# It4innovations/hyperqueue

Measured on AMD Instinct MI355X. Metric: tasks_assigned_per_sec, higher is better.
Workload: dtype u64

## Files before the change

### hyperqueue_amd/csrc/debug_capi.cpp

```cpp
#include "../../include/hqtick_debug.h"

#include <algorithm>
#include <cstring>

#include "clock_core.h"
#include "hb_order.h"
#include "milp.h"
#include "price_emul.h"

static thread_local int g_last_canonical = 0;
static thread_local long g_last_hull[2] = {0, 0};
extern "C" int hqtick_debug_milp_was_canonical(void) { return g_last_canonical; }
extern "C" void hqtick_debug_milp_last_hull(long *solves, long *nonpacking) {
    if (solves) *solves = g_last_hull[0];
    if (nonpacking) *nonpacking = g_last_hull[1];
}

extern "C" int hqtick_debug_milp_solve(int ncols, const double *obj, const uint8_t *col_kind, int nrows, const uint8_t *row_type,
                                       const double *rhs, const int *row_off, const int *row_col, const double *row_coef,
                                       double time_limit_s, int canonical, double *x_out, double *obj_out, int *is_optimal,
                                       long *nodes_out) {
    hqmilp::Model m;
    m.obj.assign(obj, obj + ncols);
    m.kind.assign(col_kind, col_kind + ncols);
// ... 38 lines not shown
    if (min_cols) emu.min_cols = min_cols;
    hqmilp::Result r = hqmilp::solve(m, time_limit_s, true, hqmilp::REFERENCE_MIP_REL_GAP, use_sweeps ? &emu : nullptr);
    g_last_canonical = r.canonical ? 1 : 0;
    g_last_hull[0] = r.hull_solves; g_last_hull[1] = r.hull_solves_nonpacking;
    if (stats_out) { stats_out[0] = r.price_sweeps; stats_out[1] = r.price_rounds; stats_out[2] = r.price_total_us; stats_out[3] = r.canonical ? 1.0 : 0.0; }
    if (!r.feasible) return 0;
    for (int j = 0; j < ncols; j++) x_out[j] = r.x[j];
    *obj_out = r.objective;
    *is_optimal = r.optimal ? 1 : 0;
    return 1;
}

static thread_local hqmilp::Probe g_block_run_probe;
extern "C" void hqtick_debug_set_block_runs(int on) {
    hqmilp::g_probe = on < 0 ? nullptr : &g_block_run_probe; hqmilp::set_block_runs(on);
    if (on >= 0) { g_block_run_probe.model = g_block_run_probe.tables = g_block_run_probe.runs = g_block_run_probe.covered = 0; }
}
extern "C" void hqtick_debug_corrupt_block_runs(int on) { g_block_run_probe.corrupt_runs = on != 0; }
extern "C" void hqtick_debug_last_coupled_digest(uint64_t out[4]) {
    out[0] = g_block_run_probe.model; out[1] = g_block_run_probe.tables; out[2] = g_block_run_probe.runs; out[3] = g_block_run_probe.covered;
}
extern "C" void hqtick_debug_set_early_sweep(int on) { hqprice::set_early_sweep(on); }
extern "C" uint32_t hqtick_debug_early_sweeps(void) { return hqprice::early_sweeps(); }
extern "C" void hqtick_debug_capture_first_cut(int on) { hqprice::capture_first_cut(on != 0); }
extern "C" uint32_t hqtick_debug_first_cut(unsigned char *out, uint32_t cap) {
    const std::vector<unsigned char> &b = hqprice::first_cut_bytes();
    if (out && cap) memcpy(out, b.data(), std::min<size_t>(cap, b.size()));
    return (uint32_t)b.size();
}

extern "C" int hqtick_debug_clock_rows(uint32_t n, const int64_t *deadline_ns, int64_t now_ns, uint32_t nv, const uint64_t *min_time_ns, int sorted_form, int64_t *remaining_out) {
    if ((n && (!deadline_ns || !remaining_out)) || (nv && !min_time_ns)) return HQTICK_E_INVALID;
    if (!sorted_form) {
        for (uint32_t w = 0; w < n; w++) {
            if (deadline_ns[w] == hqclock::NO_LIMIT) { remaining_out[w] = hqclock::NO_LIMIT; continue; }
            const int64_t r = hqclock::sat_sub(deadline_ns[w], now_ns);
            uint64_t best = 0;
            for (uint32_t v0 = 0; r >= 0 && v0 < nv; v0 += hqclock::CHUNK) best = hqclock::fold_thresholds(best, r, min_time_ns + v0, std::min(hqclock::CHUNK, nv - v0));
            remaining_out[w] = r < 0 ? -1 : (int64_t)best;
        }
        return 0;
    }
    std::vector<uint64_t> thr(min_time_ns, min_time_ns + nv);
    std::sort(thr.begin(), thr.end()); thr.erase(std::unique(thr.begin(), thr.end()), thr.end());
    for (uint32_t w = 0; w < n; w++) remaining_out[w] = hqclock::canonical_sorted(deadline_ns[w], now_ns, thr.data(), (uint32_t)thr.size());
    return 0;
// ... 4 lines not shown
```

### hyperqueue_amd/csrc/price.cpp

```cpp
#include "price.h"

#include <algorithm>
#include <chrono>
#include <cmath>
#include <cstdio>
#include <cstdlib>
#include <cstring>
#include <functional>
#include <map>
#include <numeric>

#include "lp_tab.h"
#include "milp.h"

namespace hqprice {
namespace {

using hqmilp::lp::BASIC;
using hqmilp::lp::INF;
using hqmilp::lp::LP_OPT;
using hqmilp::lp::Rows;
using hqmilp::lp::Tab;

constexpr int KMAX_HOST = 128;
constexpr int NMAX_BLOCK = 32, MMAX_BLOCK = 4;
constexpr double FIRST_PROPOSAL_SCALE = 1.0 / 16.0;
constexpr double GRID = 10000.0;
constexpr int MAX_ROUNDS = 6;
constexpr int BP_MAX_NODES = 600;
constexpr double BP_MAX_STEPS = 3.0e6;
constexpr double BP_MAX_WORK = 3.0e9;

double now_us() { return std::chrono::duration<double, std::micro>(std::chrono::steady_clock::now().time_since_epoch()).count(); }
thread_local uint32_t g_early_sweeps = 0;

struct CapRow { int flat; double rhs; std::vector<std::pair<int, double>> g; };

struct Prob {
    HostTables T;
    std::vector<int> flat_of, model_of;
    std::vector<int> gmodel;
    std::vector<double> gcost;
    int K = 0, G = 0;
    std::vector<double> h;
    std::vector<uint8_t> ge;
    std::vector<std::vector<std::pair<int, double>>> g_rows;
    std::vector<int> grp_of;
    int KG = 0;
    std::vector<int> g_off, g_col; std::vector<int32_t> g_coef;
    std::vector<int> gr_off, gr_row;
    size_t row_terms = 0;
    std::vector<CapRow> caps;
    std::vector<int32_t> base_cap;
    std::vector<int> block_of_flat;
    int n_runs = 0, run_blocks = 0;
};

// ... 179 lines not shown
    P.grp_of.assign(P.K, -1);
    std::vector<int> rep;
    for (int k = 0; k < P.K; k++) {
        int g = -1;
        for (size_t i = 0; i < rep.size() && g < 0; i++) if (sig[rep[i]] == sig[k] && wide[rep[i]].cols == wide[k].cols) g = (int)i;
        if (g < 0) { g = (int)rep.size(); rep.push_back(k); }
        P.grp_of[k] = g;
    }
    P.KG = (int)rep.size();
    if (P.KG > KMAX_HOST) return "more than 128 distinct wide left-hand sides";
    std::vector<std::vector<std::pair<int, int32_t>>> lhs((size_t)P.KG);
    for (int g = 0; g < P.KG; g++) lhs[(size_t)g] = std::move(wide[rep[g]].cols);
    finish_groups(P, lhs);
    P.base_cap = T.col_cap;
    return nullptr;
}

struct Cut {
    double cx = 0, bnd = 0; std::vector<long long> act; std::vector<double> pi;
    std::vector<uint16_t> x; bool fetched = false; std::vector<std::pair<uint32_t, int32_t>> lo;
    std::vector<double> pcx; std::vector<long long> pact;
};

struct BPNode { std::vector<int8_t> flag; std::vector<std::pair<uint32_t, int32_t>> lo, hi; double bound = INF; int depth = 0; };

struct Solver {
    const Request &rq; Sweeper &sw; Prob P;
    std::vector<Cut> cuts;
    double relaxed_bound = INF;
    std::vector<double> relaxed_pi;
    double theta_scale = 1.0;
    std::vector<double> pmax;
    bool failed = false;
    size_t cut_lo = 0;
    double work = 0.0;
    double sweep_steps = 0.0; int budget_sweeps = 0;
    int max_sweeps = 256;
    std::vector<std::pair<uint32_t, int32_t>> node_lo, node_caps; double node_cl = 0.0; std::vector<double> node_Al; bool at_root = true;
    bool base_caps = true;
    enum { EARLY_NONE = 0, EARLY_LAUNCHED, EARLY_REFUSED, EARLY_FAILED };
    int early = EARLY_NONE;
    bool early_begun = false;
    bool host_acts = false;
    double tp0 = 0.0;
    Solver(const Request &r, Sweeper &s) : rq(r), sw(s) {}

    void prepare_sweeper() {
        sw.stat_sweeps = 0; sw.stat_sweep_us = 0;
        sw.guard_s = rq.deadline_s - 0.3 * rq.time_limit_s; sw.time_up = false;
        max_sweeps = (int)std::min<size_t>(4096, std::max<size_t>(256, ((size_t)64 << 20) / ((size_t)P.T.n_cols * 2 + 1)));
    }
    void launch_on_blocks() {
        prepare_sweeper();
        const int took = sw.begin_blocks(P.T, (uint32_t)max_sweeps);
        if (took < 0) return;
        if (took == 0) { early = EARLY_REFUSED; return; }
        early_begun = true;
        const double zero = 0.0, t0 = now_us();
        sw.pending_k = 0;
        if (!sw.sweep_launch(&zero)) { early = EARLY_FAILED; return; }
        sw.stat_sweep_us += now_us() - t0;
        early = EARLY_LAUNCHED; host_acts = true; g_early_sweeps++;
        if (rq.trace) fprintf(stderr, "[price] first sweep (prices 0) launched on the block tables at %.3f ms\n", (now_us() - tp0) / 1e3);
    }
    bool activities_from_patterns(uint32_t sweep, SweepTotals &tot) {
        const HostTables &T = P.T;
        const uint16_t *x = sw.patterns(sweep, 1);
// ... 231 lines not shown
                for (size_t k = cut_lo; k < cuts.size(); k++) for (int p = 0; p < NP; p++) {
                    const double l = lam[k * PARTS + p];
                    if (l == 0.0) continue;
                    const long long *pa = &cuts[k].pact[(size_t)p * K];
                    for (int r = 0; r < K; r++) colact[r] += l * (double)pa[r];
                }
                auto keep = std::move(probe); probe = nullptr;
                const bool go = keep(colact, lb_master);
                probe = std::move(keep);
                if (go) return false;
            }
            bool same = !pi_prev_master.empty();
            for (int i = 0; i < KL && same; i++) same = std::fabs(mt.x[i] - pi_prev_master[i]) <= 1e-15 + 1e-12 * std::fabs(mt.x[i]);
            pi_prev_master.assign(mt.x.begin(), mt.x.begin() + KL);
            const double alpha = (it < 3 || same) ? 0.0 : 0.3;
            for (int k = 0; k < K; k++) pi[k] = alpha * pi_best[k];
            for (int i = 0; i < KL; i++) pi[lk[i]] += (1.0 - alpha) * mt.x[i];
            if (it == 0 && cut_lo == 0 && cuts.size() == 1) {
                std::vector<double> pa;
                static const bool agg_on = !(getenv("HQPRICE_AGG_START") && atoi(getenv("HQPRICE_AGG_START")) == 0);
                if (agg_on && aggregate_prices(hB, lk, pa)) { pi = pa; if (rq.trace) fprintf(stderr, "[price]   first proposal: the duals of the model aggregated over chunks of blocks\n"); }
                else for (int k = 0; k < K; k++) pi[k] *= FIRST_PROPOSAL_SCALE;
            }
            const int ci = evaluate(pi);
            if (ci < 0) break;
            if (sw.time_up) { if (rq.trace) fprintf(stderr, "[price] 70 %% of the time limit gone inside the master loop\n"); return false; }
            if (budget_sweeps >= 8) { if (rq.trace) fprintf(stderr, "[price] blocks keep running out of their search budget (%d sweeps): not a model for the sweeps\n", budget_sweeps); return false; }
            const double L = fixed_value(cuts[ci], hB, cB);
            if (L < ub_best) { ub_best = L; pi_best = pi; }
            push_cuts(&mt);
        }
        if (!converged) {
            if (mt.solve(200000) != LP_OPT) return false;
            lb_master = -mt.objective() * theta_scale + cB;
            if (ub_best - lb_master > 1e-3 * std::fabs(ub_best)) { if (rq.trace) fprintf(stderr, "[price] master not converged: %.9f vs %.9f\n", ub_best, lb_master); return false; }
        }
        multipliers(lambda);
        if (rq.trace) fprintf(stderr, "[price]   master: %d priced rows + %d parts, %d cut rows, %ld pivots, %.1f us inside the LP (%d active rows)\n", KL, NP, M.m, mt.iters, lp_us, mt.ma);
        pi_out.assign(K, 0.0);
        for (int i = 0; i < KL; i++) pi_out[lk[i]] = mt.x[i];
        *bound_out = ub_best;
        if (no_sweeps) { settled.valid = true; settled.hB = hB; settled.cB = cB; settled.lambda = lambda; settled.pi = pi_out; settled.bound = ub_best; settled.n_cuts = cuts.size(); settled.cut_lo = cut_lo; }
        return true;
    }

    bool fetch_patterns() {
        size_t first = cuts.size();
        for (size_t k = 0; k < cuts.size(); k++) if (!cuts[k].fetched) { first = k; break; }
        if (first == cuts.size()) return true;
        const uint32_t count = (uint32_t)(cuts.size() - first);
        const uint16_t *pat = sw.patterns((uint32_t)first, count);
        if (!pat) { failed = true; return false; }
        const uint32_t nc = P.T.n_cols;
        for (uint32_t i = 0; i < count; i++) {
            Cut &c = cuts[first + i];
            if (c.fetched) continue;
            c.x.assign(pat + (size_t)i * nc, pat + (size_t)(i + 1) * nc);
            for (auto &l : c.lo) c.x[l.first] = (uint16_t)(c.x[l.first] + l.second);
            c.fetched = true;
        }
        return true;
    }

    std::vector<uint16_t> round_patterns(const std::vector<double> &lambda, const std::vector<double> &pi, const std::vector<double> &hB,
                                         const std::vector<char> *usable = nullptr, const std::vector<int32_t> *lo_of = nullptr, int variant = 0) {
        const int K = P.K; const HostTables &T = P.T;
        const uint32_t S = (uint32_t)cuts.size();
        const double t_r0 = now_us();
        if (!fetch_patterns()) return {};
        auto pat_of = [&](int k) { return cuts[(size_t)k].x.data(); };
        const uint32_t per = (T.n_blocks + PARTS - 1) / PARTS;
        auto lam = [&](int k, uint32_t p) { return lambda[(size_t)k * PARTS + p]; };
        std::vector<int> active;
        for (uint32_t k = 0; k < S; k++) {
            if (usable && !(*usable)[k]) continue;
            bool any = false; for (uint32_t p = 0; p < (uint32_t)PARTS && !any; p++) any = lam((int)k, p) > 1e-9;
            if (any) active.push_back((int)k);
        }
        if (active.empty()) return {};
        const int Q = (int)active.size();
        std::vector<double> lpact(K, 0.0), wgt(K);
        for (int k : active) {
            const Cut &c = cuts[k];
            if (c.pact.empty()) { for (int r = 0; r < K; r++) lpact[r] += lam(k, 0) * (double)c.act[r]; continue; }
            for (uint32_t p = 0; p < (uint32_t)PARTS; p++) { const double l = lam(k, p); if (l > 0.0) for (int r = 0; r < K; r++) lpact[r] += l * (double)c.pact[(size_t)p * P.K + r]; }
        }
        for (int r = 0; r < K; r++) {
            const bool tight = pi[r] > 1e-12 || hB[r] - lpact[r] <= 1e-6 * std::max(1.0, std::fabs(hB[r]));
            wgt[r] = (tight ? 1.0 : 0.02) / std::max(1.0, std::fabs(hB[r]));
        }
        auto block_act = [&](uint32_t b, const uint16_t *x, std::vector<double> &out) {
            double ga[KMAX_HOST];
            for (int g = 0; g < P.KG; g++) ga[g] = 0.0;
            for (uint32_t f = T.blk_off[b]; f < T.blk_off[b + 1]; f++) { const uint16_t xv = x[f]; if (!xv) continue; for (uint32_t e = T.col_woff[f]; e < T.col_woff[f + 1]; e++) ga[T.w_row[e]] += (double)T.w_coef[e] * (double)xv; }
            for (int r = 0; r < K; r++) out[r] = ga[P.grp_of[r]];
        };
        std::vector<uint16_t> x(T.n_cols, 0);
        std::vector<double> cum(K, 0.0);
        std::vector<int> chosen(T.n_blocks, 0);
        {
            const int KG = P.KG;
            std::vector<double> wg(KG, 0.0), cumg(KG, 0.0), tgtg(KG, 0.0), candg((size_t)Q * KG);
            for (int r = 0; r < K; r++) wg[P.grp_of[r]] += wgt[r];
            std::vector<char> on(Q); std::vector<const double *> cgp(Q, nullptr);
            for (uint32_t bi = 0; bi < T.n_blocks; bi++) {
                const uint32_t b = variant == 1 ? T.n_blocks - 1 - bi : bi;
                const uint32_t part = b / per;
                int first = -1; bool all_same = true;
                const size_t blk_bytes = (size_t)(T.blk_off[b + 1] - T.blk_off[b]) * 2;
                for (int q = 0; q < Q; q++) {
                    const double l = lam(active[q], part);
                    on[q] = l > 1e-9;
                    if (!on[q]) continue;
                    const uint16_t *px = pat_of(active[q]);
                    if (first >= 0 && memcmp(px + T.blk_off[b], pat_of(active[first]) + T.blk_off[b], blk_bytes) == 0) cgp[q] = cgp[first];
                    else {
                        if (first < 0) first = q; else all_same = false;
                        double *cg = &candg[(size_t)q * KG];
                        for (int g = 0; g < KG; g++) cg[g] = 0.0;
                        for (uint32_t f = T.blk_off[b]; f < T.blk_off[b + 1]; f++) { const uint16_t xv = px[f]; if (!xv) continue; for (uint32_t e = T.col_woff[f]; e < T.col_woff[f + 1]; e++) cg[T.w_row[e]] += (double)T.w_coef[e] * (double)xv; }
                        cgp[q] = cg;
                    }
                    const double *cg = cgp[q];
                    for (int g = 0; g < KG; g++) tgtg[g] += l * cg[g];
                }
                int bq = -1; double be = INF;
                if (all_same) bq = first;
                else for (int q = 0; q < Q; q++) {
                    if (!on[q]) continue;
                    const double *cg = cgp[q];
                    double e = 0.0;
                    for (int g = 0; g < KG; g++) e += std::fabs(cumg[g] + cg[g] - tgtg[g]) * wg[g];
                    if (e < be - 1e-15) { be = e; bq = q; }
                }
                if (bq < 0) return {};
                const double *cb = cgp[bq];
                for (int g = 0; g < KG; g++) cumg[g] += cb[g];
                chosen[b] = active[bq];
                memcpy(&x[T.blk_off[b]], pat_of(active[bq]) + T.blk_off[b], (size_t)(T.blk_off[b + 1] - T.blk_off[b]) * 2);
            }
            for (int r = 0; r < K; r++) cum[r] = cumg[P.grp_of[r]];
        }
        if (rq.trace) fprintf(stderr, "[price]   rounding: diffusion done at %.3f us, %d active cuts\n", now_us() - t_r0, Q);
        auto ge_short = [&](const std::vector<double> &c) { double s = 0.0; for (int r = 0; r < K; r++) if (P.ge[r] && c[r] > hB[r] + 1e-9) s += c[r] - hB[r]; return s; };
        if (ge_short(cum) > 0.0) {
            std::vector<int> pool = active;
            for (int k = (int)S - 1; k >= 0 && (int)pool.size() < Q + 12; k--) if ((!usable || (*usable)[k]) && std::find(pool.begin(), pool.end(), k) == pool.end()) pool.push_back(k);
            std::vector<double> a0(K), a1(K), c2(K);
            double cmax = 0.0; for (double c : T.col_cost) cmax = std::max(cmax, c);
            struct Cand { double score; uint32_t b; int k; };
            std::vector<Cand> cl; std::vector<double> colshort, coltight;
            auto evaluate_switch = [&](uint32_t b, int k, double v0, double &score) {
                const uint16_t *px = pat_of(k);
                block_act(b, px, a1);
                double gain = 0.0, newviol = 0.0;
                for (int r = 0; r < K; r++) {
                    if (a0[r] == a1[r]) continue;
                    const double c = cum[r] - a0[r] + a1[r];
                    if (P.ge[r]) gain += std::max(0.0, cum[r] - hB[r]) - std::max(0.0, c - hB[r]);
                    else newviol += std::max(0.0, c - hB[r]) - std::max(0.0, cum[r] - hB[r]);
                }
                if (!(gain > 1e-9)) return false;
                double v1 = 0.0; for (uint32_t f = T.blk_off[b]; f < T.blk_off[b + 1]; f++) v1 += T.col_cost[f] * (double)px[f];
                score = gain * 10.0 * cmax - (v0 - v1) - std::max(0.0, newviol) * cmax;
                return true;
            };
            auto value_of = [&](uint32_t b) { double v = 0.0; for (uint32_t f = T.blk_off[b]; f < T.blk_off[b + 1]; f++) v += T.col_cost[f] * (double)x[f]; return v; };
            for (int pass = 0; pass < 64 && ge_short(cum) > 0.0; pass++) {
                const double base = ge_short(cum);
                cl.clear();
                std::vector<int> short_in(P.KG, 0);
                for (int r = 0; r < K; r++) if (P.ge[r] && cum[r] > hB[r] + 1e-9) short_in[P.grp_of[r]]++;
                std::vector<int> tight_in(P.KG, 0);
                double spare = 0.0;
                for (int r = 0; r < K; r++) if (P.ge[r] && cum[r] <= hB[r] + 1e-9 && hB[r] - cum[r] <= 2.0 + 1e-9) { tight_in[P.grp_of[r]]++; spare += std::max(0.0, hB[r] - cum[r]); }
                colshort.assign(T.n_cols, 0.0); coltight.assign(T.n_cols, 0.0);
                for (uint32_t f = 0; f < T.n_cols; f++) for (uint32_t e = T.col_woff[f]; e < T.col_woff[f + 1]; e++) {
                    const int ns = short_in[T.w_row[e]], nt = tight_in[T.w_row[e]];
                    if (ns) colshort[f] += (double)ns * (double)T.w_coef[e];
                    if (nt) coltight[f] += (double)nt * (double)T.w_coef[e];
                }
                for (uint32_t b = 0; b < T.n_blocks; b++) {
                    for (int k : pool) {
                        if (k == chosen[b]) continue;
                        const uint16_t *px = pat_of(k);
                        double gain = 0.0, dv = 0.0, dmg = 0.0; bool differs = false;
                        for (uint32_t f = T.blk_off[b]; f < T.blk_off[b + 1]; f++) {
                            const int d = (int)px[f] - (int)x[f];
                            if (!d) continue;
                            differs = true; dv += T.col_cost[f] * (double)d;
                            gain -= colshort[f] * (double)d;
                            dmg += coltight[f] * (double)d;
                        }
                        if (!differs || !(gain - std::max(0.0, dmg - spare) > 1e-9)) continue;
                        cl.push_back({std::min(gain, base) * 10.0 * cmax + dv, b, k});
                    }
                }
                if (rq.trace) fprintf(stderr, "[price]     pass %d: short by %.1f, %zu candidate switches, at %.3f us\n", pass, base, cl.size(), now_us() - t_r0);
                if (cl.empty()) break;
                const size_t top = std::min<size_t>(cl.size(), 512);
                std::partial_sort(cl.begin(), cl.begin() + (long)top, cl.end(), [](const Cand &p, const Cand &q) { return p.score > q.score || (p.score == q.score && (p.b < q.b || (p.b == q.b && p.k < q.k))); });
                cl.resize(top);
                std::vector<char> moved(T.n_blocks, 0);
                for (const Cand &cd : cl) {
                    if (!(ge_short(cum) > 0.0)) break;
                    if (moved[cd.b]) continue;
                    {
                        const uint16_t *px = pat_of(cd.k); double gain = 0.0;
                        for (uint32_t f = T.blk_off[cd.b]; f < T.blk_off[cd.b + 1]; f++) {
                            const int d = (int)px[f] - (int)x[f];
                            if (d) for (uint32_t e = T.col_woff[f]; e < T.col_woff[f + 1]; e++) { const int g = T.w_row[e]; for (int q = P.gr_off[g]; q < P.gr_off[g + 1]; q++) { const int r = P.gr_row[q]; if (P.ge[r] && cum[r] > hB[r] + 1e-9) gain -= (double)T.w_coef[e] * (double)d; } }
                        }
                        if (!(gain > 1e-9)) continue;
                    }
                    block_act(cd.b, pat_of(chosen[cd.b]), a0);
                    double score;
                    if (!evaluate_switch(cd.b, cd.k, value_of(cd.b), score)) continue;
                    for (int r = 0; r < K; r++) cum[r] += a1[r] - a0[r];
                    chosen[cd.b] = cd.k; moved[cd.b] = 1;
                    memcpy(&x[T.blk_off[cd.b]], pat_of(cd.k) + T.blk_off[cd.b], (size_t)(T.blk_off[cd.b + 1] - T.blk_off[cd.b]) * 2);
                }
                if (ge_short(cum) >= base - 1e-9) break;
            }
            if (ge_short(cum) > 0.0) return {};
        }
        if (rq.trace) fprintf(stderr, "[price]   rounding: >= repair done at %.3f us\n", now_us() - t_r0);
        for (int r = 0; r < K; r++) {
            if (cum[r] <= hB[r] + 1e-9) continue;
            std::vector<int> cols;
            const int gr = P.grp_of[r];
            for (int k = P.g_off[gr]; k < P.g_off[gr + 1]; k++) if (P.g_coef[k] > 0 && x[P.g_col[k]] > 0) cols.push_back(k);
            std::sort(cols.begin(), cols.end(), [&](int a, int b) { const double ca = T.col_cost[P.g_col[a]] / P.g_coef[a], cb = T.col_cost[P.g_col[b]] / P.g_coef[b]; return ca < cb || (ca == cb && a > b); });
            for (int k : cols) {
                const int f = P.g_col[k];
                while (x[f] > (lo_of ? (uint16_t)(*lo_of)[f] : 0) && cum[r] > hB[r] + 1e-9) {
                    bool ok = true;
                    for (uint32_t e = T.col_woff[f]; e < T.col_woff[f + 1] && ok; e++) if (T.w_coef[e] < 0) { const int g = T.w_row[e]; for (int q = P.gr_off[g]; q < P.gr_off[g + 1] && ok; q++) if (cum[P.gr_row[q]] - (double)T.w_coef[e] > hB[P.gr_row[q]] + 1e-9) ok = false; }
                    if (!ok) break;
                    x[f]--;
                    for (uint32_t e = T.col_woff[f]; e < T.col_woff[f + 1]; e++) { const int g = T.w_row[e]; for (int q = P.gr_off[g]; q < P.gr_off[g + 1]; q++) cum[P.gr_row[q]] -= (double)T.w_coef[e]; }
                }
                if (cum[r] <= hB[r] + 1e-9) break;
            }
            if (cum[r] > hB[r] + 1e-9) return {};
        }
        return x;
    }

    struct NodeLP { double bound = INF; bool pruned = false; std::vector<double> lambda, pi, bfrac; };

    bool apply_node(const BPNode &nd, std::vector<int32_t> &lo_arr, std::vector<int32_t> &hi_arr) {
// ... 893 lines not shown
    S.tp0 = tp0;
    if (g_capture_cut) g_first_cut.clear();
    std::vector<double> ub, c; double cmax = 1.0;
    const std::function<void()> hook = [&S]() { S.launch_on_blocks(); };
    if (const char *why = build_from_model(mv, S.P, ub, c, cmax, early_sweep_on() ? &hook : nullptr)) {
        if (S.early_begun) sw.end();
        Answer ans; ans.why = why; return ans;
    }
    if (cost_scale) *cost_scale = cmax;
    Polisher pol(S.P, mv.n);
    rq.polish = [&pol](std::vector<double> &x, double &value) { return pol.run(x, value); };
    return run_solver(S, tp0);
}

void flatten_for_probe(const ModelView &mv, bool trace) {
    Prob P; std::vector<double> ub, c; double cmax = 1.0;
    const char *why = build_from_model(mv, P, ub, c, cmax);
    if (trace) fprintf(stderr, "[price] flattened for the probe alone: %s\n", why ? why : "tables built");
}

void set_check_hints(bool on) { g_check_hints = on; g_hint_mismatches = 0; }
void set_early_sweep(int on) { g_early_sweep = on; g_early_sweeps = 0; }
uint32_t early_sweeps() { return g_early_sweeps; }
void capture_first_cut(bool on) { g_capture_cut = on; g_first_cut.clear(); }
const std::vector<unsigned char> &first_cut_bytes() { return g_first_cut; }
int hint_mismatches() { return g_hint_mismatches; }

Answer solve(const Request &rq, Sweeper &sw) {
    Solver S(rq, sw);
    const double tp0 = now_us();
    if (const char *why = build(rq, S.P)) { Answer ans; ans.why = why; return ans; }
    return run_solver(S, tp0);
}

}
```

### hyperqueue_amd/csrc/price.h

```cpp
#pragma once
#include <cstdint>
#include <functional>
#include <vector>

namespace hqprice {

struct HostTables {
    uint32_t n_blocks = 0, n_cols = 0, K = 0;
    std::vector<uint32_t> blk_off; std::vector<uint8_t> blk_m; std::vector<double> blk_cap;
    std::vector<double> col_cost, col_a; std::vector<int32_t> col_cap; std::vector<uint32_t> col_woff; std::vector<uint16_t> w_row; std::vector<int32_t> w_coef;
};

struct SweepTotals {
    double cx = 0, rc = 0, bnd = 0;
    uint32_t n_budget = 0, max_steps = 0;
    std::vector<long long> act;
    std::vector<double> part_cx;
    std::vector<long long> part_act;
};
constexpr int PARTS = 16;

struct RangeValues { const double *cx = nullptr, *rc = nullptr, *bnd = nullptr; const uint32_t *steps = nullptr; const long long *part_act = nullptr; };

void totals_from_blocks(uint32_t n_blocks, uint32_t K, const double *cx, const double *rc, const double *bnd, const uint32_t *steps, const long long *part_act, SweepTotals &out);

struct Sweeper {
    virtual ~Sweeper() {}
    virtual bool begin(const HostTables &t, uint32_t max_sweeps) = 0;
    virtual int begin_blocks(const HostTables &t, uint32_t max_sweeps) { (void)t; (void)max_sweeps; return -1; }
    virtual bool begin_wide() { return false; }
    virtual bool set_caps(const int32_t *col_cap) = 0;
    virtual bool set_block_caps(const double *blk_cap) = 0;
    virtual bool sweep(const double *pi, SweepTotals &out) = 0;
    virtual bool sweep_launch(const double *pi) { pending_pi.assign(pi, pi + pending_k); return true; }
    virtual bool sweep_finish(SweepTotals &out) { return sweep(pending_pi.data(), out); }
    std::vector<double> pending_pi; uint32_t pending_k = 0;
    virtual const uint16_t *patterns(uint32_t first, uint32_t count) = 0;
    virtual void end() = 0;
    virtual bool sweep_range(const double *pi, uint32_t b0, uint32_t b1, RangeValues &out) { (void)pi; (void)b0; (void)b1; (void)out; return false; }
    double guard_s = 1e300;
    bool time_up = false;
    virtual bool merges_clock() const { return false; }
    uint32_t min_cols = 256;
    uint32_t budget = 4096;
    uint32_t stat_sweeps = 0;
    double stat_sweep_us = 0;
};

struct Request {
    int n = 0, m = 0;
    const int *roff = nullptr, *rcol = nullptr; const double *rcoef = nullptr, *rlo = nullptr, *rhi = nullptr;
    const double *row_scale = nullptr; const uint8_t *row_implied = nullptr;
    const int32_t *col_group = nullptr;
    const double *c = nullptr, *ub = nullptr;
    const double *incumbent = nullptr; double incumbent_value = 0.0;
    double rel_gap = 1e-4;
    double time_limit_s = 5.0;
    double deadline_s = 1e300;
    std::function<bool(std::vector<double> &x, double &value)> polish;
    bool trace = false;
// ... 8 lines not shown
    const char *why = "";
    std::vector<int> block_of; std::vector<double> block_value, rcost;
};

Answer solve(const Request &rq, Sweeper &sw);

struct ModelView {
    int n = 0, m = 0;
    const double *obj = nullptr; const uint8_t *kind = nullptr;
    const uint8_t *rtype = nullptr; const double *rhs = nullptr;
    const int *roff = nullptr, *rcol = nullptr; const double *rcoef = nullptr;
    const int32_t *col_group = nullptr; const uint8_t *row_implied = nullptr;
    const int32_t *row_lhs = nullptr, *row_lhs_len = nullptr;
    const int *list_off = nullptr, *list_col = nullptr; int n_lists = 0;
    const int32_t *row_block = nullptr; const uint32_t *col_ub = nullptr;
    const int32_t *block_runs = nullptr; int n_block_runs = 0;
    uint64_t *run_stats = nullptr;
    uint64_t *tables_digest = nullptr;
};
void set_check_hints(bool on);
int hint_mismatches();
void set_early_sweep(int on);
uint32_t early_sweeps();
void capture_first_cut(bool on);
const std::vector<unsigned char> &first_cut_bytes();
void flatten_for_probe(const ModelView &mv, bool trace);
Answer solve_model(const ModelView &mv, double rel_gap, double time_limit_s, double deadline_s, bool trace, Sweeper &sw, double *cost_scale);

struct Exchange {
    uint32_t rank = 0, world = 1;
    virtual ~Exchange() {}
    virtual bool allgather(const void *send, void *recv, size_t bytes) = 0;
    uint64_t n_calls = 0, n_bytes = 0; double us = 0;
};

struct ShardedSweeper : Sweeper {
    Sweeper &inner; Exchange &ex;
    const HostTables *T = nullptr;
    std::vector<uint32_t> rank_b0, rank_b1, rank_p0, rank_p1;
    uint32_t max_blocks = 0, max_parts = 0, max_cols = 0;
    std::vector<unsigned char> send, recv;
    std::vector<double> cx, rc, bnd; std::vector<uint32_t> steps; std::vector<long long> part_act;
    std::vector<uint16_t> pats;
    uint32_t n_sweeps = 0;
    uint32_t min_blocks = 1025;
    bool pass = false;
// ... 12 lines not shown
```

### hyperqueue_amd/csrc/price_dev.h

```cpp
#pragma once
#include <hip/hip_runtime.h>

#include <cstdlib>

#include "devbuf.h"
#include "price.h"

namespace hqprice {

struct DeviceSweeper : Sweeper {
    hipStream_t stream = nullptr;
    hqbuf::PinBuf h_stage, h_res, h_pats, h_pin, h_prof, h_blkv;
    static constexpr uint32_t PIN_SWEEPS = 64;
    bool sync_clean = false;
    bool in_flight = false; double flight_t0 = 0; uint32_t flight_blocks = 0;
    bool profile = getenv("HQTICK_PRICE_PROFILE") != nullptr; double prof_med[16] = {0}, prof_max[16] = {0}, prof_steps = 0, prof_span = 0, prof_tail = 0; int prof_n = 0;
    hqbuf::DevBuf d_tab, d_pats, d_blk, d_sync, d_prof;
    const HostTables *T = nullptr;
    size_t o_off = 0, o_m = 0, o_cap = 0, o_cost = 0, o_a = 0, o_ccap = 0, o_woff = 0, o_wrow = 0, o_wcoef = 0, tab_bytes = 0;
    bool blocks_only = false;
    uint32_t flight_k = 0;
    size_t wide_room = 0;
    uint32_t n_sweeps = 0, cap_sweeps = 0, seq = 0;
    uint32_t max_block_cols = 0;
    bool force_nmax = getenv("HQTICK_PRICE_NMAX") != nullptr;
    int force_waves = getenv("HQTICK_PRICE_WAVES") ? atoi(getenv("HQTICK_PRICE_WAVES")) : 0;
    uint32_t dbg = getenv("HQTICK_PRICE_DBG") ? (uint32_t)atoi(getenv("HQTICK_PRICE_DBG")) : 0u;
    double last_kernel_us = 0;
    uint64_t total_sweeps = 0, total_block_solves = 0; double total_us = 0;
    explicit DeviceSweeper(hipStream_t s) : stream(s) {}
    ~DeviceSweeper() override;
    bool begin(const HostTables &t, uint32_t max_sweeps) override;
    int begin_blocks(const HostTables &t, uint32_t max_sweeps) override;
    bool begin_wide() override;
    bool size_buffers(const HostTables &t, uint32_t max_sweeps);
    void stage_blocks(const HostTables &t);
    bool set_caps(const int32_t *col_cap) override;
    bool set_block_caps(const double *blk_cap) override;
    bool sweep(const double *pi, SweepTotals &out) override;
    bool sweep_range(const double *pi, uint32_t b0, uint32_t b1, RangeValues &out) override;
    bool launch(const double *pi, uint32_t b0, uint32_t b1, bool local, SweepTotals *out);
    bool launch_only(const double *pi, uint32_t b0, uint32_t b1, bool local);
    bool wait_done(SweepTotals *out);
    bool sweep_launch(const double *pi) override;
    bool sweep_finish(SweepTotals &out) override;
    const uint16_t *patterns(uint32_t first, uint32_t count) override;
    void end() override;
};

}
```

### hyperqueue_amd/csrc/price_emul.h

```cpp
#pragma once
#include <algorithm>
#include <vector>

#include "price.h"

namespace hqprice {

struct EmulatedSweeper : Sweeper {
    const HostTables *T = nullptr;
    std::vector<int32_t> caps;
    std::vector<double> bcaps;
    std::vector<uint16_t> pats;
    std::vector<double> blk_cx, blk_rc, blk_bnd;
    std::vector<uint32_t> blk_steps;
    std::vector<long long> slots;
    uint32_t n_sweeps = 0, cap_sweeps = 0;
    int fail_at = -1;
    bool blocks_only = false, held_there = false;
    std::vector<uint32_t> zero_woff;
    SweepTotals held;
    bool begin(const HostTables &t, uint32_t max_sweeps) override;
    int begin_blocks(const HostTables &t, uint32_t max_sweeps) override;
    bool begin_wide() override;
    bool sweep_launch(const double *pi) override;
    bool sweep_finish(SweepTotals &out) override;
    bool set_caps(const int32_t *col_cap) override;
    bool set_block_caps(const double *blk_cap) override;
    bool sweep(const double *pi, SweepTotals &out) override;
    bool sweep_range(const double *pi, uint32_t b0, uint32_t b1, RangeValues &out) override;
    const uint16_t *patterns(uint32_t first, uint32_t count) override;
    void end() override;
};

}
```

### include/hqtick_debug.h

```cpp
#ifndef HQTICK_DEBUG_H
#define HQTICK_DEBUG_H
#include <stdint.h>
#include "hqtick.h"
#ifdef __cplusplus
extern "C" {
#endif
#if defined(__GNUC__)
#pragma GCC visibility push(default)
#endif

int hqtick_debug_milp_solve(int ncols, const double *obj, const uint8_t *col_kind, int nrows, const uint8_t *row_type,
                            const double *rhs, const int *row_off, const int *row_col, const double *row_coef,
                            double time_limit_s, int canonical, double *x_out, double *obj_out, int *is_optimal,
                            long *nodes_out);

int hqtick_debug_last_order(const hqtick_ctx *ctx, uint32_t *n_runs, uint32_t *n_levels, double *order_us);

int hqtick_debug_last_scan(const hqtick_ctx *ctx, int which, uint32_t *n_levels, uint32_t *n_groups, uint32_t shape[4],
                           uint64_t *levels, uint32_t cap_levels, uint32_t *hist, uint32_t cap_groups);

int hqtick_debug_order_view(hqtick_ctx *ctx, uint32_t n_requests, uint32_t counts[4], uint32_t *perm, uint32_t *inv, uint32_t *lrank, uint64_t cap_slots, uint32_t *run_rq,
                            uint32_t *run_start, uint32_t *run_rank, uint64_t *run_prio, uint32_t cap_runs);
int hqtick_debug_order_select(hqtick_ctx *ctx, const uint32_t *rq_sel_base, const uint32_t *q_tnc, uint32_t n_sel, int mark_mode, uint64_t *sel_task, uint32_t *sel_rank,
                              uint32_t *rq_after, uint32_t *err);
// ... 12 lines not shown
void hqtick_debug_map_order_u32(const uint32_t *keys, uint32_t n, uint32_t *out_pos);

int hqtick_debug_block_solve_host(uint32_t n_cols, uint32_t n_resources, const uint32_t *ent_off, const uint32_t *ent_res, const uint8_t *ent_kind,
                                  const uint64_t *ent_amount, const uint32_t *weight, const double *pool, uint32_t n_classes, const uint64_t *free_,
                                  const uint64_t *total, const uint64_t *elig, uint32_t budget, uint32_t *x, uint32_t *status, uint32_t *steps);
void hqtick_debug_set_block_emulation(int on, uint32_t budget);
void hqtick_debug_last_stage_us(double *out3);
void hqtick_debug_last_blocks(uint32_t *n_emulated, uint32_t *n_host);

int hqtick_time_kernel(hqtick_ctx *ctx, int which, int iters, double *avg_us);
int hqtick_timeline(const hqtick_ctx *ctx, double *out, int cap);
const uint64_t *hqtick_block_profile_last(const hqtick_ctx *ctx, uint32_t *n_classes);


void hqtick_debug_set_price_emulation(int on, uint32_t min_cols);
void hqtick_debug_set_price_fault(int fail_at);
void hqtick_debug_set_fast_path(int on);
void hqtick_debug_check_model_hints(int on);
int hqtick_debug_model_hint_mismatches(void);
void hqtick_debug_set_block_runs(int on);
void hqtick_debug_last_coupled_digest(uint64_t out[4]);
void hqtick_debug_set_early_sweep(int on);
uint32_t hqtick_debug_early_sweeps(void);
void hqtick_debug_capture_first_cut(int on);
uint32_t hqtick_debug_first_cut(unsigned char *out, uint32_t cap);
void hqtick_debug_corrupt_block_runs(int on);
void hqtick_debug_last_price(uint32_t *sweeps, uint32_t *rounds);
uint32_t hqtick_debug_last_mn(const uint32_t **rq, const uint32_t **off, const uint32_t **worker);
int hqtick_debug_milp_solve_priced(int ncols, const double *obj, const uint8_t *col_kind, const int32_t *col_group, int nrows, const uint8_t *row_type,
                                   const uint8_t *row_implied, const double *rhs, const int *row_off, const int *row_col, const double *row_coef,
                                   double time_limit_s, int use_sweeps, uint32_t min_cols, double *x_out, double *obj_out, int *is_optimal, double *stats_out);

struct hqwire_tables;
struct hqwire_records;
struct hqwire_output;
int hqwire_debug_encode_host(const struct hqwire_tables *tables, const struct hqwire_records *records, const struct hqwire_output *out);
int hqwire_debug_encode_host_order(const struct hqwire_tables *tables, const struct hqwire_records *records, const struct hqwire_output *out, int order);
struct hqwire_table;
struct hqwire_table_config;
int hqwire_debug_table_create_host(struct hqwire_table **out, const struct hqwire_table_config *cfg, int order);

void hqtick_debug_set_block_guard(uint32_t verify, uint32_t tick_seq, int corrupt_mode, uint32_t corrupt_class, uint32_t corrupt_fill);
void hqtick_debug_last_block_guard(uint32_t *verified, uint32_t *mismatch, uint32_t *rejected);
void hqtick_debug_set_block_memo(int on);
uint32_t hqtick_debug_last_block_memo(void);
void hqtick_debug_set_exchange(hqtick_exchange_fn fn, void *user, uint32_t rank, uint32_t world, uint32_t min_blocks, uint32_t min_classes);
// ... 15 lines not shown
```

Baseline: 73.34 million.

## Precompute per-block cut activity tables while sweeps are in flight for rounding

Each cut's per-block group activities and costs are computed on the host while a device pricing sweep is in flight. Blocks whose pattern matches an older cut share one stored row. The rounding and repair passes then use these tables: they look up rows, skip pairs that share a pattern, and compute gain from group rows instead of per-column loops. Scratch vectors are reused across passes. This adds host memory, capped by a byte limit, and more bookkeeping, and the overlap only pays off when rounding dominates.

Result: slower. 71.46 million (-2.6%).

```diff
diff --git a/hyperqueue_amd/csrc/debug_capi.cpp b/hyperqueue_amd/csrc/debug_capi.cpp
--- a/hyperqueue_amd/csrc/debug_capi.cpp
+++ b/hyperqueue_amd/csrc/debug_capi.cpp
@@ -84,6 +84,12 @@
 }
 extern "C" void hqtick_debug_set_early_sweep(int on) { hqprice::set_early_sweep(on); }
 extern "C" uint32_t hqtick_debug_early_sweeps(void) { return hqprice::early_sweeps(); }
+extern "C" void hqtick_debug_set_round_prep(int on) { hqprice::set_round_prep(on); }
+extern "C" void hqtick_debug_set_round_prep_limit(uint64_t limit_bytes) { hqprice::set_round_prep_limit(limit_bytes); }
+extern "C" void hqtick_debug_round_prep_stats(uint64_t out[5]) {
+    const hqprice::RoundPrepStats &st = hqprice::round_prep_stats();
+    out[0] = st.in_flight; out[1] = st.at_rounding; out[2] = st.pairs_skipped; out[3] = st.lookups; out[4] = st.unprepared;
+}
 extern "C" void hqtick_debug_capture_first_cut(int on) { hqprice::capture_first_cut(on != 0); }
 extern "C" uint32_t hqtick_debug_first_cut(unsigned char *out, uint32_t cap) {
     const std::vector<unsigned char> &b = hqprice::first_cut_bytes();
diff --git a/hyperqueue_amd/csrc/price.cpp b/hyperqueue_amd/csrc/price.cpp
--- a/hyperqueue_amd/csrc/price.cpp
+++ b/hyperqueue_amd/csrc/price.cpp
@@ -1,6 +1,7 @@
 #include "price.h"
 
 #include <algorithm>
+#include <cassert>
 #include <chrono>
 #include <cmath>
 #include <cstdio>
@@ -33,6 +34,12 @@
 
 double now_us() { return std::chrono::duration<double, std::micro>(std::chrono::steady_clock::now().time_since_epoch()).count(); }
 thread_local uint32_t g_early_sweeps = 0;
+constexpr uint64_t ROUND_PREP_BYTES = (uint64_t)32 << 20;
+thread_local int g_round_prep = -1; thread_local uint64_t g_round_prep_limit = 0; thread_local RoundPrepStats g_prep_stats;
+bool round_prep_on() {
+    static const bool env_on = !(getenv("HQPRICE_ROUND_PREP") && atoi(getenv("HQPRICE_ROUND_PREP")) == 0);
+    return g_round_prep < 0 ? env_on : g_round_prep != 0;
+}
 
 struct CapRow { int flat; double rhs; std::vector<std::pair<int, double>> g; };
 
@@ -258,6 +265,13 @@
     std::vector<double> pcx; std::vector<long long> pact;
 };
 
+struct CutPrep {
+    bool ready = false, refused = false;
+    std::vector<uint32_t> cls, row, older;
+    std::vector<double> val;
+    std::vector<double> ga;
+};
+
 struct BPNode { std::vector<int8_t> flag; std::vector<std::pair<uint32_t, int32_t>> lo, hi; double bound = INF; int depth = 0; };
 
 struct Solver {
@@ -279,6 +293,15 @@
     bool early_begun = false;
     bool host_acts = false;
     double tp0 = 0.0;
+    const bool prep_on = round_prep_on();
+    const uint64_t prep_limit = g_round_prep_limit ? g_round_prep_limit : ROUND_PREP_BYTES;
+    std::vector<CutPrep> prep;
+    std::vector<uint32_t> last_cls;
+    uint64_t prep_bytes = 0; size_t flight_next = 0;
+    std::vector<std::pair<size_t, const uint16_t *>> flight_pats;
+    struct Cand { double score; uint32_t b; int k; };
+    std::vector<Cand> r_cl; std::vector<double> r_colshort, r_coltight; std::vector<char> r_moved; std::vector<int> r_short_in, r_tight_in;
+    std::vector<std::pair<int, double>> r_gs, r_gt;
     Solver(const Request &r, Sweeper &s) : rq(r), sw(s) {}
 
     void prepare_sweeper() {
@@ -556,7 +579,7 @@
                 if (agg_on && aggregate_prices(hB, lk, pa)) { pi = pa; if (rq.trace) fprintf(stderr, "[price]   first proposal: the duals of the model aggregated over chunks of blocks\n"); }
                 else for (int k = 0; k < K; k++) pi[k] *= FIRST_PROPOSAL_SCALE;
             }
-            const int ci = evaluate(pi);
+            const int ci = evaluate_preparing(pi);
             if (ci < 0) break;
             if (sw.time_up) { if (rq.trace) fprintf(stderr, "[price] 70 %% of the time limit gone inside the master loop\n"); return false; }
             if (budget_sweeps >= 8) { if (rq.trace) fprintf(stderr, "[price] blocks keep running out of their search budget (%d sweeps): not a model for the sweeps\n", budget_sweeps); return false; }
@@ -577,6 +600,61 @@
         if (no_sweeps) { settled.valid = true; settled.hB = hB; settled.cB = cB; settled.lambda = lambda; settled.pi = pi_out; settled.bound = ub_best; settled.n_cuts = cuts.size(); settled.cut_lo = cut_lo; }
         return true;
     }
+
+    bool prepare_cut(size_t k, const uint16_t *pat, bool flight) {
+        if (prep.size() < cuts.size()) prep.resize(cuts.size());
+        CutPrep &pp = prep[k];
+        if (pp.ready || pp.refused) return pp.ready;
+        const HostTables &T = P.T;
+        const size_t KG = (size_t)P.KG, nb = T.n_blocks;
+        if (prep_bytes + nb * (20 + 8 * KG) > prep_limit) { pp.refused = true; g_prep_stats.unprepared++; return false; }
+        Cut &c = cuts[k];
+        const double t0 = rq.trace ? now_us() : 0.0;
+        if (!c.fetched) {
+            if (!pat) return false;
+            c.x.assign(pat, pat + T.n_cols);
+            for (auto &l : c.lo) c.x[l.first] = (uint16_t)(c.x[l.first] + l.second);
+            c.fetched = true;
+        }
+        const uint16_t *x = c.x.data();
+        if (last_cls.size() != nb) last_cls.assign(nb, ~0u);
+        pp.cls.resize(nb); pp.row.resize(nb); pp.older.resize(nb); pp.val.resize(nb);
+        uint32_t n_own = 0;
+        for (uint32_t b = 0; b < nb; b++) {
+            const uint32_t f0 = T.blk_off[b]; const size_t bytes = (size_t)(T.blk_off[b + 1] - f0) * 2;
+            uint32_t j = last_cls[b];
+            while (j != ~0u && memcmp(x + f0, cuts[j].x.data() + f0, bytes) != 0) j = prep[j].older[b];
+            if (j != ~0u) { pp.cls[b] = j; pp.row[b] = prep[j].row[b]; pp.val[b] = prep[j].val[b]; continue; }
+            pp.cls[b] = (uint32_t)k; pp.row[b] = n_own++; pp.older[b] = last_cls[b]; last_cls[b] = (uint32_t)k;
+        }
+        pp.ga.assign((size_t)n_own * KG, 0.0);
+        const uint32_t *woff = T.col_woff.data(); const uint16_t *wr = T.w_row.data(); const int32_t *wc = T.w_coef.data();
+        for (uint32_t b = 0; b < nb; b++) {
+            if (pp.cls[b] != (uint32_t)k) continue;
+            double *cg = &pp.ga[(size_t)pp.row[b] * KG]; double v = 0.0;
+            for (uint32_t f = T.blk_off[b]; f < T.blk_off[b + 1]; f++) { const uint16_t xv = x[f]; if (!xv) continue; for (uint32_t e = woff[f]; e < woff[f + 1]; e++) cg[wr[e]] += (double)wc[e] * (double)xv; }
+            for (uint32_t f = T.blk_off[b]; f < T.blk_off[b + 1]; f++) v += T.col_cost[f] * (double)x[f];
+            pp.val[b] = v;
+        }
+        prep_bytes += nb * 20 + (uint64_t)n_own * KG * 8;
+        pp.ready = true;
+        if (flight) g_prep_stats.in_flight++; else g_prep_stats.at_rounding++;
+        if (rq.trace) fprintf(stderr, "[price]   cut %zu prepared for the rounding in %.1f us (%s), %u of %zu blocks with a pattern of their own\n", k, now_us() - t0, flight ? "a sweep in flight" : "at rounding time", n_own, nb);
+        return true;
+    }
+    int evaluate_preparing(const std::vector<double> &pi) {
+        if (!prep_on) return evaluate(pi);
+        flight_pats.clear();
+        for (const size_t e = std::min<size_t>(cuts.size(), sw.patterns_in_place()); flight_next < e; flight_next++) {
+            const uint16_t *pat = cuts[flight_next].fetched ? nullptr : sw.patterns((uint32_t)flight_next, 1);
+            if (pat || cuts[flight_next].fetched) flight_pats.push_back({flight_next, pat});
+        }
+        if (!evaluate_launch(pi)) return -1;
+        for (auto &fp : flight_pats) prepare_cut(fp.first, fp.second, true);
+        return evaluate(pi, true);
+    }
+    const CutPrep *prep_of(int k) const { return prep_on && (size_t)k < prep.size() && prep[(size_t)k].ready ? &prep[(size_t)k] : nullptr; }
+    const double *prep_row(const CutPrep *pp, uint32_t b) const { return &prep[pp->cls[b]].ga[(size_t)pp->row[b] * (size_t)P.KG]; }
 
     bool fetch_patterns() {
         size_t first = cuts.size();
@@ -602,6 +680,8 @@
         const uint32_t S = (uint32_t)cuts.size();
         const double t_r0 = now_us();
         if (!fetch_patterns()) return {};
+        if (prep_on) for (size_t k = 0; k < cuts.size(); k++) prepare_cut(k, nullptr, false);
+        struct Served { uint64_t skipped = 0, lookups = 0; ~Served() { g_prep_stats.pairs_skipped += skipped; g_prep_stats.lookups += lookups; } } served;
         auto pat_of = [&](int k) { return cuts[(size_t)k].x.data(); };
         const uint32_t per = (T.n_blocks + PARTS - 1) / PARTS;
         auto lam = [&](int k, uint32_t p) { return lambda[(size_t)k * PARTS + p]; };
@@ -629,14 +709,22 @@
             for (uint32_t f = T.blk_off[b]; f < T.blk_off[b + 1]; f++) { const uint16_t xv = x[f]; if (!xv) continue; for (uint32_t e = T.col_woff[f]; e < T.col_woff[f + 1]; e++) ga[T.w_row[e]] += (double)T.w_coef[e] * (double)xv; }
             for (int r = 0; r < K; r++) out[r] = ga[P.grp_of[r]];
         };
+        auto cut_act = [&](uint32_t b, int k, std::vector<double> &out) {
+            const CutPrep *pk = prep_of(k);
+            if (!pk) { block_act(b, pat_of(k), out); return; }
+            const double *ga = prep_row(pk, b); served.lookups++;
+            for (int r = 0; r < K; r++) out[r] = ga[P.grp_of[r]];
+        };
         std::vector<uint16_t> x(T.n_cols, 0);
         std::vector<double> cum(K, 0.0);
         std::vector<int> chosen(T.n_blocks, 0);
+        bool x_is_chosen = true;
         {
             const int KG = P.KG;
             std::vector<double> wg(KG, 0.0), cumg(KG, 0.0), tgtg(KG, 0.0), candg((size_t)Q * KG);
             for (int r = 0; r < K; r++) wg[P.grp_of[r]] += wgt[r];
             std::vector<char> on(Q); std::vector<const double *> cgp(Q, nullptr);
+            std::vector<const CutPrep *> pq(Q); for (int q = 0; q < Q; q++) pq[q] = prep_of(active[q]);
             for (uint32_t bi = 0; bi < T.n_blocks; bi++) {
                 const uint32_t b = variant == 1 ? T.n_blocks - 1 - bi : bi;
                 const uint32_t part = b / per;
@@ -647,8 +735,11 @@
                     on[q] = l > 1e-9;
                     if (!on[q]) continue;
                     const uint16_t *px = pat_of(active[q]);
-                    if (first >= 0 && memcmp(px + T.blk_off[b], pat_of(active[first]) + T.blk_off[b], blk_bytes) == 0) cgp[q] = cgp[first];
-                    else {
+                    if (first >= 0 && (pq[q] && pq[first] ? pq[q]->cls[b] == pq[first]->cls[b] : memcmp(px + T.blk_off[b], pat_of(active[first]) + T.blk_off[b], blk_bytes) == 0)) cgp[q] = cgp[first];
+                    else if (pq[q]) {
+                        if (first < 0) first = q; else all_same = false;
+                        cgp[q] = prep_row(pq[q], b); served.lookups++;
+                    } else {
                         if (first < 0) first = q; else all_same = false;
                         double *cg = &candg[(size_t)q * KG];
                         for (int g = 0; g < KG; g++) cg[g] = 0.0;
@@ -675,18 +766,20 @@
             }
             for (int r = 0; r < K; r++) cum[r] = cumg[P.grp_of[r]];
         }
-        if (rq.trace) fprintf(stderr, "[price]   rounding: diffusion done at %.3f us, %d active cuts\n", now_us() - t_r0, Q);
+        if (rq.trace) fprintf(stderr, "[price]   rounding: diffusion done at %.3f us, %d active cuts%s\n", now_us() - t_r0, Q, variant == 1 ? " (blocks in reverse order)" : "");
         auto ge_short = [&](const std::vector<double> &c) { double s = 0.0; for (int r = 0; r < K; r++) if (P.ge[r] && c[r] > hB[r] + 1e-9) s += c[r] - hB[r]; return s; };
         if (ge_short(cum) > 0.0) {
             std::vector<int> pool = active;
             for (int k = (int)S - 1; k >= 0 && (int)pool.size() < Q + 12; k--) if ((!usable || (*usable)[k]) && std::find(pool.begin(), pool.end(), k) == pool.end()) pool.push_back(k);
             std::vector<double> a0(K), a1(K), c2(K);
             double cmax = 0.0; for (double c : T.col_cost) cmax = std::max(cmax, c);
-            struct Cand { double score; uint32_t b; int k; };
-            std::vector<Cand> cl; std::vector<double> colshort, coltight;
+            std::vector<Cand> &cl = r_cl; std::vector<double> &colshort = r_colshort, &coltight = r_coltight;
+            std::vector<char> &moved = r_moved; std::vector<int> &short_in = r_short_in, &tight_in = r_tight_in;
+            std::vector<const CutPrep *> ppool(pool.size()); bool pool_prepared = true;
+            for (size_t i = 0; i < pool.size(); i++) { ppool[i] = prep_of(pool[i]); pool_prepared = pool_prepared && ppool[i]; }
             auto evaluate_switch = [&](uint32_t b, int k, double v0, double &score) {
                 const uint16_t *px = pat_of(k);
-                block_act(b, px, a1);
+                cut_act(b, k, a1);
                 double gain = 0.0, newviol = 0.0;
                 for (int r = 0; r < K; r++) {
                     if (a0[r] == a1[r]) continue;
@@ -695,39 +788,72 @@
                     else newviol += std::max(0.0, c - hB[r]) - std::max(0.0, cum[r] - hB[r]);
                 }
                 if (!(gain > 1e-9)) return false;
-                double v1 = 0.0; for (uint32_t f = T.blk_off[b]; f < T.blk_off[b + 1]; f++) v1 += T.col_cost[f] * (double)px[f];
+                double v1 = 0.0;
+                if (const CutPrep *pk = prep_of(k)) { v1 = pk->val[b]; served.lookups++; }
+                else for (uint32_t f = T.blk_off[b]; f < T.blk_off[b + 1]; f++) v1 += T.col_cost[f] * (double)px[f];
                 score = gain * 10.0 * cmax - (v0 - v1) - std::max(0.0, newviol) * cmax;
                 return true;
             };
-            auto value_of = [&](uint32_t b) { double v = 0.0; for (uint32_t f = T.blk_off[b]; f < T.blk_off[b + 1]; f++) v += T.col_cost[f] * (double)x[f]; return v; };
+            auto value_of = [&](uint32_t b) {
+                if (const CutPrep *pc = prep_of(chosen[b])) { served.lookups++; return pc->val[b]; }
+                double v = 0.0; for (uint32_t f = T.blk_off[b]; f < T.blk_off[b + 1]; f++) v += T.col_cost[f] * (double)x[f]; return v;
+            };
             for (int pass = 0; pass < 64 && ge_short(cum) > 0.0; pass++) {
                 const double base = ge_short(cum);
                 cl.clear();
-                std::vector<int> short_in(P.KG, 0);
+                short_in.assign(P.KG, 0);
                 for (int r = 0; r < K; r++) if (P.ge[r] && cum[r] > hB[r] + 1e-9) short_in[P.grp_of[r]]++;
-                std::vector<int> tight_in(P.KG, 0);
+                tight_in.assign(P.KG, 0);
                 double spare = 0.0;
                 for (int r = 0; r < K; r++) if (P.ge[r] && cum[r] <= hB[r] + 1e-9 && hB[r] - cum[r] <= 2.0 + 1e-9) { tight_in[P.grp_of[r]]++; spare += std::max(0.0, hB[r] - cum[r]); }
-                colshort.assign(T.n_cols, 0.0); coltight.assign(T.n_cols, 0.0);
-                for (uint32_t f = 0; f < T.n_cols; f++) for (uint32_t e = T.col_woff[f]; e < T.col_woff[f + 1]; e++) {
-                    const int ns = short_in[T.w_row[e]], nt = tight_in[T.w_row[e]];
-                    if (ns) colshort[f] += (double)ns * (double)T.w_coef[e];
-                    if (nt) coltight[f] += (double)nt * (double)T.w_coef[e];
-                }
-                for (uint32_t b = 0; b < T.n_blocks; b++) {
-                    for (int k : pool) {
-                        if (k == chosen[b]) continue;
-                        const uint16_t *px = pat_of(k);
-                        double gain = 0.0, dv = 0.0, dmg = 0.0; bool differs = false;
-                        for (uint32_t f = T.blk_off[b]; f < T.blk_off[b + 1]; f++) {
-                            const int d = (int)px[f] - (int)x[f];
-                            if (!d) continue;
-                            differs = true; dv += T.col_cost[f] * (double)d;
-                            gain -= colshort[f] * (double)d;
-                            dmg += coltight[f] * (double)d;
+                assert(x_is_chosen);
+                if (pool_prepared) {
+                    r_gs.clear(); r_gt.clear();
+                    for (int g = 0; g < P.KG; g++) { if (short_in[g]) r_gs.push_back({g, (double)short_in[g]}); if (tight_in[g]) r_gt.push_back({g, (double)tight_in[g]}); }
+                    for (uint32_t b = 0; b < T.n_blocks; b++) {
+                        const CutPrep *pc = prep_of(chosen[b]);
+                        const uint32_t cb = pc->cls[b];
+                        const double *ac = prep_row(pc, b);
+                        for (size_t pi_ = 0; pi_ < pool.size(); pi_++) {
+                            const int k = pool[pi_];
+                            if (k == chosen[b]) continue;
+                            if (ppool[pi_]->cls[b] == cb) { served.skipped++; continue; }
+                            const double *ak = prep_row(ppool[pi_], b); served.lookups++;
+                            double gain = 0.0, dmg = 0.0;
+                            for (auto &t : r_gs) gain -= t.second * (ak[t.first] - ac[t.first]);
+                            for (auto &t : r_gt) dmg += t.second * (ak[t.first] - ac[t.first]);
+                            if (!(gain - std::max(0.0, dmg - spare) > 1e-9)) continue;
+                            const uint16_t *px = pat_of(k); double dv = 0.0;
+                            for (uint32_t f = T.blk_off[b]; f < T.blk_off[b + 1]; f++) { const int d = (int)px[f] - (int)x[f]; if (d) dv += T.col_cost[f] * (double)d; }
+                            cl.push_back({std::min(gain, base) * 10.0 * cmax + dv, b, k});
                         }
-                        if (!differs || !(gain - std::max(0.0, dmg - spare) > 1e-9)) continue;
-                        cl.push_back({std::min(gain, base) * 10.0 * cmax + dv, b, k});
+                    }
+                } else {
+                    colshort.assign(T.n_cols, 0.0); coltight.assign(T.n_cols, 0.0);
+                    for (uint32_t f = 0; f < T.n_cols; f++) for (uint32_t e = T.col_woff[f]; e < T.col_woff[f + 1]; e++) {
+                        const int ns = short_in[T.w_row[e]], nt = tight_in[T.w_row[e]];
+                        if (ns) colshort[f] += (double)ns * (double)T.w_coef[e];
+                        if (nt) coltight[f] += (double)nt * (double)T.w_coef[e];
+                    }
+                    for (uint32_t b = 0; b < T.n_blocks; b++) {
+                        const CutPrep *pc = prep_of(chosen[b]);
+                        const uint32_t cb = pc ? pc->cls[b] : 0;
+                        for (size_t pi_ = 0; pi_ < pool.size(); pi_++) {
+                            const int k = pool[pi_];
+                            if (k == chosen[b]) continue;
+                            if (pc && ppool[pi_] && ppool[pi_]->cls[b] == cb) { served.skipped++; continue; }
+                            const uint16_t *px = pat_of(k);
+                            double gain = 0.0, dv = 0.0, dmg = 0.0; bool differs = false;
+                            for (uint32_t f = T.blk_off[b]; f < T.blk_off[b + 1]; f++) {
+                                const int d = (int)px[f] - (int)x[f];
+                                if (!d) continue;
+                                differs = true; dv += T.col_cost[f] * (double)d;
+                                gain -= colshort[f] * (double)d;
+                                dmg += coltight[f] * (double)d;
+                            }
+                            if (!differs || !(gain - std::max(0.0, dmg - spare) > 1e-9)) continue;
+                            cl.push_back({std::min(gain, base) * 10.0 * cmax + dv, b, k});
+                        }
                     }
                 }
                 if (rq.trace) fprintf(stderr, "[price]     pass %d: short by %.1f, %zu candidate switches, at %.3f us\n", pass, base, cl.size(), now_us() - t_r0);
@@ -735,7 +861,7 @@
                 const size_t top = std::min<size_t>(cl.size(), 512);
                 std::partial_sort(cl.begin(), cl.begin() + (long)top, cl.end(), [](const Cand &p, const Cand &q) { return p.score > q.score || (p.score == q.score && (p.b < q.b || (p.b == q.b && p.k < q.k))); });
                 cl.resize(top);
-                std::vector<char> moved(T.n_blocks, 0);
+                moved.assign(T.n_blocks, 0);
                 for (const Cand &cd : cl) {
                     if (!(ge_short(cum) > 0.0)) break;
                     if (moved[cd.b]) continue;
@@ -747,7 +873,7 @@
                         }
                         if (!(gain > 1e-9)) continue;
                     }
-                    block_act(cd.b, pat_of(chosen[cd.b]), a0);
+                    cut_act(cd.b, chosen[cd.b], a0);
                     double score;
                     if (!evaluate_switch(cd.b, cd.k, value_of(cd.b), score)) continue;
                     for (int r = 0; r < K; r++) cum[r] += a1[r] - a0[r];
@@ -759,8 +885,10 @@
             if (ge_short(cum) > 0.0) return {};
         }
         if (rq.trace) fprintf(stderr, "[price]   rounding: >= repair done at %.3f us\n", now_us() - t_r0);
+        x_is_chosen = false; (void)x_is_chosen;
         for (int r = 0; r < K; r++) {
             if (cum[r] <= hB[r] + 1e-9) continue;
+            if (rq.trace) fprintf(stderr, "[price]   rounding: <= repair of row %d, over by %.1f\n", r, cum[r] - hB[r]);
             std::vector<int> cols;
             const int gr = P.grp_of[r];
             for (int k = P.g_off[gr]; k < P.g_off[gr + 1]; k++) if (P.g_coef[k] > 0 && x[P.g_col[k]] > 0) cols.push_back(k);
@@ -1700,6 +1828,9 @@
 void set_check_hints(bool on) { g_check_hints = on; g_hint_mismatches = 0; }
 void set_early_sweep(int on) { g_early_sweep = on; g_early_sweeps = 0; }
 uint32_t early_sweeps() { return g_early_sweeps; }
+void set_round_prep(int on) { g_round_prep = on; g_prep_stats = RoundPrepStats(); }
+void set_round_prep_limit(uint64_t limit_bytes) { g_round_prep_limit = limit_bytes; }
+const RoundPrepStats &round_prep_stats() { return g_prep_stats; }
 void capture_first_cut(bool on) { g_capture_cut = on; g_first_cut.clear(); }
 const std::vector<unsigned char> &first_cut_bytes() { return g_first_cut; }
 int hint_mismatches() { return g_hint_mismatches; }
diff --git a/hyperqueue_amd/csrc/price.h b/hyperqueue_amd/csrc/price.h
--- a/hyperqueue_amd/csrc/price.h
+++ b/hyperqueue_amd/csrc/price.h
@@ -36,6 +36,7 @@
     virtual bool sweep_finish(SweepTotals &out) { return sweep(pending_pi.data(), out); }
     std::vector<double> pending_pi; uint32_t pending_k = 0;
     virtual const uint16_t *patterns(uint32_t first, uint32_t count) = 0;
+    virtual uint32_t patterns_in_place() const { return 0; }
     virtual void end() = 0;
     virtual bool sweep_range(const double *pi, uint32_t b0, uint32_t b1, RangeValues &out) { (void)pi; (void)b0; (void)b1; (void)out; return false; }
     double guard_s = 1e300;
@@ -90,6 +91,10 @@
 int hint_mismatches();
 void set_early_sweep(int on);
 uint32_t early_sweeps();
+void set_round_prep(int on);
+void set_round_prep_limit(uint64_t limit_bytes);
+struct RoundPrepStats { uint64_t in_flight = 0, at_rounding = 0, pairs_skipped = 0, lookups = 0, unprepared = 0; };
+const RoundPrepStats &round_prep_stats();
 void capture_first_cut(bool on);
 const std::vector<unsigned char> &first_cut_bytes();
 void flatten_for_probe(const ModelView &mv, bool trace);
diff --git a/hyperqueue_amd/csrc/price_dev.h b/hyperqueue_amd/csrc/price_dev.h
--- a/hyperqueue_amd/csrc/price_dev.h
+++ b/hyperqueue_amd/csrc/price_dev.h
@@ -45,6 +45,7 @@
     bool sweep_launch(const double *pi) override;
     bool sweep_finish(SweepTotals &out) override;
     const uint16_t *patterns(uint32_t first, uint32_t count) override;
+    uint32_t patterns_in_place() const override { return PIN_SWEEPS; }
     void end() override;
 };
 
diff --git a/hyperqueue_amd/csrc/price_emul.h b/hyperqueue_amd/csrc/price_emul.h
--- a/hyperqueue_amd/csrc/price_emul.h
+++ b/hyperqueue_amd/csrc/price_emul.h
@@ -29,6 +29,7 @@
     bool sweep(const double *pi, SweepTotals &out) override;
     bool sweep_range(const double *pi, uint32_t b0, uint32_t b1, RangeValues &out) override;
     const uint16_t *patterns(uint32_t first, uint32_t count) override;
+    uint32_t patterns_in_place() const override { return 64; }
     void end() override;
 };
 
diff --git a/include/hqtick_debug.h b/include/hqtick_debug.h
--- a/include/hqtick_debug.h
+++ b/include/hqtick_debug.h
@@ -58,6 +58,9 @@
 void hqtick_debug_last_coupled_digest(uint64_t out[4]);
 void hqtick_debug_set_early_sweep(int on);
 uint32_t hqtick_debug_early_sweeps(void);
+void hqtick_debug_set_round_prep(int on);
+void hqtick_debug_set_round_prep_limit(uint64_t limit_bytes);
+void hqtick_debug_round_prep_stats(uint64_t out[5]);
 void hqtick_debug_capture_first_cut(int on);
 uint32_t hqtick_debug_first_cut(unsigned char *out, uint32_t cap);
 void hqtick_debug_corrupt_block_runs(int on);
```
